# fani-lab/OpeNTF

Measured on AMD Instinct MI355X. Metric: teams/sec (train) bnn_emb d=128 on DBLP, higher is better.
Workload: dtype f32 (fp16x3 split products, f32 accumulate)

## Files before the change

opentf_amd/csrc/ntf_fused_dw.hip:

```cpp
#include "ntf_fused_common.h"

namespace ntf {

struct DwArgs {
    int B, M, Bpad;
    const float *__restrict__ dzT, *__restrict__ h, *__restrict__ hs, *__restrict__ mu, *__restrict__ rho;
    const float* wp;
    const uint32_t* sbits; int nCB; uint32_t so_k0, so_k1; int so_inj;
    float *__restrict__ g_mu, *__restrict__ g_rho, *__restrict__ g_b, *__restrict__ g_bp;
    float klw;
    float *__restrict__ w_mu, *__restrict__ w_rho, *__restrict__ m_mu, *__restrict__ v_mu, *__restrict__ m_rho, *__restrict__ v_rho;
    float lr_over_bc1, b1, b2, eps, bc2_sqrt;
    int wg_begin;
    int* rflag; int rmode;
    const uint32_t* sT;
    const uint32_t* sinT;
    const uint16_t* hb;
    float a_scale, unscale;
    int ksplit; float* part; int64_t slab; int part_row0;
    unsigned long long* stamps;
    int Hr;
    int ntile, stagger;
    NormalSpec cur_eps; int lean;
    int produce; NormalSpec nx_eps; float* nx_wp; uint16_t *nx_pl_wp, *nx_pl_mu; float nx_pscale; double nx_klw; double* nx_kl; int* nx_rflag;
};

__device__ __forceinline__ float adam_update(float p, float g, float& m, float& v, float lr_over_bc1, float b1, float b2, float eps, float bc2_sqrt) {
    adam_step(p, g, m, v, lr_over_bc1, b1, b2, eps, __builtin_amdgcn_rcpf(bc2_sqrt));
    return p;
}

__device__ __forceinline__ uint32_t transpose32(uint32_t a, int il) {
    uint32_t m = 0x0000FFFFu;
#pragma unroll
    for (int j = 16; j != 0; j >>= 1) {
        const uint32_t pv = (uint32_t)__shfl_xor((int)a, j, 64);
        const bool lower = (il & j) == 0;
        const uint32_t lo = lower ? a : pv, hi = lower ? pv : a;
        const uint32_t t = ((lo >> j) ^ hi) & m;
        a ^= lower ? (t << j) : t;
        m ^= m << (j >> 1);
    }
    return a;
}

__device__ __forceinline__ void dw_produce_next(const DwArgs& p, int64_t idx0, const float (&mu4)[4], const float (&rho4)[4], float& kl, float& amax) {
    float z[4], ov[4];
#if defined(DWQ_ABL) && (DWQ_ABL & 2)
    z[0] = z[1] = z[2] = z[3] = 1.f;
#else
    normal4(p.nx_eps, idx0 >> 2, idx0, INT64_MAX, z);
#endif
#pragma unroll
    for (int j = 0; j < 4; ++j) {
        float ls;
        const float sigma = softplus_rho_fast(rho4[j], ls);
        ov[j] = sigma * z[j];
        kl += -ls + 0.5f * (sigma * sigma + mu4[j] * mu4[j]) - 0.5f;
    }
    if (!p.lean) *reinterpret_cast<float4*>(p.nx_wp + idx0) = make_float4(ov[0], ov[1], ov[2], ov[3]);
    const int64_t row = idx0 >> 7; const int j = (int)(idx0 & 127);
    amax = fmaxf(amax, fmaxf(fmaxf(fabsf(ov[0]), fabsf(ov[1])), fmaxf(fabsf(ov[2]), fabsf(ov[3]))));
    amax = fmaxf(amax, fmaxf(fmaxf(fabsf(mu4[0]), fabsf(mu4[1])), fmaxf(fabsf(mu4[2]), fabsf(mu4[3]))));
    planes_store_quad(p.nx_pl_wp, row, j, 128, ov[0], ov[1], ov[2], ov[3], p.nx_pscale);
    planes_store_quad(p.nx_pl_mu, row, j, 128, mu4[0], mu4[1], mu4[2], mu4[3], p.nx_pscale);
}
__device__ __forceinline__ void dw_produce_next_fnn(const DwArgs& p, int64_t idx0, const float (&mu4)[4], float& amax) {
    const int64_t row = idx0 >> 7; const int j = (int)(idx0 & 127);
    amax = fmaxf(amax, fmaxf(fmaxf(fabsf(mu4[0]), fabsf(mu4[1])), fmaxf(fabsf(mu4[2]), fabsf(mu4[3]))));
    planes_store_quad(p.nx_pl_mu, row, j, 128, mu4[0], mu4[1], mu4[2], mu4[3], p.nx_pscale);
}
template <bool BAYES = true>
__device__ __forceinline__ void dw_produce_finish(const DwArgs& p, float kl, float amax, double* red, int nwaves) {
    if (!(amax * p.nx_pscale <= 65504.f)) *p.nx_rflag = 1;
    if (!BAYES) return;
    const double s = wave_reduce_sum_d((double)kl);
    __syncthreads();
    if ((threadIdx.x & 63) == 0) red[threadIdx.x >> 6] = s;
    __syncthreads();
    if (threadIdx.x == 0) { double t = 0.0; for (int w = 0; w < nwaves; ++w) t += red[w]; atomicAdd(p.nx_kl, t * p.nx_klw); }
}

template <int H, bool BAYES, bool ADAM, int HG = H, bool PAD = false>
__device__ __forceinline__ void out_dw_f32_body(const DwArgs& p, char* smem, int jh = 0) {
    constexpr int NJT = H / 32;
    constexpr int KB = 32;
    constexpr int HROW = 4 * H;
    constexpr int TA = DW_TC * KB * 4;
    constexpr int TH = KB * HROW;
    constexpr int STAGE = TA + (BAYES ? 2 : 1) * TH;
    const int tid = threadIdx.x, lane = tid & 63, wave = tid >> 6, il = lane & 31, half = lane >> 5;
    if (range_guard_skip(p.rflag, p.rmode, false)) return;
    const int c0 = (p.wg_begin + blockIdx.x) * DW_TC;
    const int crow = wave * 32 + il;
    const int c = c0 + crow;
    const int nib = p.Bpad / KB;

    f32x16 acc1[NJT], acc2[NJT];
#pragma unroll
    for (int j = 0; j < NJT; ++j)
#pragma unroll
        for (int r = 0; r < 16; ++r) { acc1[j][r] = 0.f; acc2[j][r] = 0.f; }
    float sum1 = 0.f, sum2 = 0.f;

    const uint32_t smem_base = lds_addr(smem);
    const int wave_u = __builtin_amdgcn_readfirstlane(wave);
    auto stage = [&](int ib, int buf) {
        const uint32_t sb = smem_base + buf * STAGE;
#pragma unroll
        for (int n = 0; n < TA / 1024 / DW_WAVES; ++n) {
            const int inst = wave_u * (TA / 1024 / DW_WAVES) + n;
            const int row = inst * 8 + (lane >> 3), pch = lane & 7;
            const int q = pch ^ ((row >> 1) & 7);
            glds16(p.dzT + ((int64_t)(c0 >> 8) * nib + ib) * 8192 + row * 32 + 4 * q, sb + inst * 1024);
        }
        constexpr int HI = TH / 1024;
#pragma unroll
        for (int n = 0; n < (HI + DW_WAVES - 1) / DW_WAVES; ++n) {
            const int inst = wave_u * ((HI + DW_WAVES - 1) / DW_WAVES) + n;
            if (inst < HI) {
                int64_t goff = (int64_t)ib * KB * H + inst * 256 + lane * 4;
                if constexpr (HG != H) { const int f = inst * 256 + lane * 4; goff = (int64_t)(ib * KB + f / H) * HG + jh * H + f % H; }
                glds16(p.h + goff, sb + TA + inst * 1024);
                if (BAYES) glds16(p.hs + goff, sb + TA + TH + inst * 1024);
            }
        }
    };

    const uint32_t cb = (uint32_t)((c0 + wave * 32) >> 5);
    auto sign_col_word = [&](int ib) -> uint32_t {
        const int i = ib * KB + il;
        uint32_t w = 0u;
        if (p.so_inj) { if ((int)cb < p.nCB) w = p.sbits[(int64_t)i * p.nCB + cb]; }
        else w = sign_word(p.so_k0, p.so_k1, (uint32_t)i, cb);
        return transpose32(w, il);
    };
    uint32_t word_next = 0;
    if (BAYES) word_next = sign_col_word(0);
    stage(0, 0);
    asm volatile("s_waitcnt vmcnt(0)" ::: "memory");
    __syncthreads();
    for (int ib = 0; ib < nib; ++ib) {
        const int buf = ib & 1;
        const uint32_t word = word_next >> (4 * half);
        if (BAYES && ib + 1 < nib) word_next = sign_col_word(ib + 1);
        if (ib + 1 < nib) stage(ib + 1, buf ^ 1);
        const char* sA = smem + buf * STAGE;
        const char* sH = sA + TA;
#pragma unroll
        for (int t = 0; t < 4; ++t) {
            const int q = 2 * t + half;
            const float4 a = *reinterpret_cast<const float4*>(sA + crow * 128 + 16 * (q ^ ((crow >> 1) & 7)));
            const float av[4] = {a.x, a.y, a.z, a.w};
#pragma unroll
            for (int e4 = 0; e4 < 4; ++e4) {
                const int kk = 8 * t + e4;
                const float a1 = av[e4];
                sum1 += a1;
                float a2 = a1;
                if (BAYES) { a2 = __uint_as_float(__float_as_uint(a1) ^ ((word << (31 - kk)) & 0x80000000u)); sum2 += a2; }
                const char* hb = sH + (kk + 4 * half) * HROW + 4 * NJT * il;
                float bv[NJT], bsv[NJT];
                if (NJT == 4) {
                    const float4 b4 = *reinterpret_cast<const float4*>(hb); bv[0] = b4.x; bv[1] = b4.y; bv[NJT > 2 ? 2 : 0] = b4.z; bv[NJT > 3 ? 3 : 0] = b4.w;
                    if (BAYES) { const float4 s4 = *reinterpret_cast<const float4*>(hb + TH); bsv[0] = s4.x; bsv[1] = s4.y; bsv[NJT > 2 ? 2 : 0] = s4.z; bsv[NJT > 3 ? 3 : 0] = s4.w; }
                } else if (NJT == 2) {
                    const float2 b2 = *reinterpret_cast<const float2*>(hb); bv[0] = b2.x; bv[NJT > 1 ? 1 : 0] = b2.y;
                    if (BAYES) { const float2 s2 = *reinterpret_cast<const float2*>(hb + TH); bsv[0] = s2.x; bsv[NJT > 1 ? 1 : 0] = s2.y; }
                } else {
                    bv[0] = *reinterpret_cast<const float*>(hb);
                    if (BAYES) bsv[0] = *reinterpret_cast<const float*>(hb + TH);
                }
#pragma unroll
                for (int jt = 0; jt < NJT; ++jt) {
                    acc1[jt] = __builtin_amdgcn_mfma_f32_32x32x2f32(a1, bv[jt], acc1[jt], 0, 0, 0);
                    if (BAYES) acc2[jt] = __builtin_amdgcn_mfma_f32_32x32x2f32(a2, bsv[jt], acc2[jt], 0, 0, 0);
                }
            }
        }
        asm volatile("s_waitcnt vmcnt(0)" ::: "memory");
        __syncthreads();
    }

    sum1 += __shfl_xor(sum1, 32, 64);
    sum2 += __shfl_xor(sum2, 32, 64);
    if (half == 0 && c < p.M && jh == 0) { p.g_b[c] = sum1; if (BAYES) p.g_bp[c] = sum2; }

    float nx_kl = 0.f, nx_amax = 0.f;
    const int ldw = PAD ? p.Hr : HG;
    const bool lane_live = !PAD || jh * H + NJT * il < p.Hr;
#pragma unroll
    for (int r = 0; r < 16; ++r) {
        const int cr = c0 + wave * 32 + rowmap(r, half);
        if (cr >= p.M || !lane_live) continue;
        const int64_t idx0 = (int64_t)cr * ldw + jh * H + NJT * il;
        float gm[NJT], gr[NJT], pm[NJT], pr[NJT];
#pragma unroll
        for (int jt = 0; jt < NJT; ++jt) {
            pm[jt] = ADAM ? p.w_mu[idx0 + jt] : (BAYES ? p.mu[idx0 + jt] : 0.f);
            if (!BAYES) { gm[jt] = acc1[jt][r]; gr[jt] = 0.f; pr[jt] = 0.f; }
            else {
                const float rh = ADAM ? p.w_rho[idx0 + jt] : p.rho[idx0 + jt], w = p.wp[idx0 + jt];
                pr[jt] = rh;
                const RhoTerms t = rho_terms(rh);
                gm[jt] = acc1[jt][r] + p.klw * pm[jt];
                gr[jt] = (t.lo ? acc2[jt][r] * w : acc2[jt][r] * (w / t.sigma) * t.sg) + p.klw * t.kl_a * t.kl_b;
            }
        }
        if (!ADAM) {
#pragma unroll
            for (int jt = 0; jt < NJT; ++jt) { p.g_mu[idx0 + jt] = gm[jt]; if (BAYES) p.g_rho[idx0 + jt] = gr[jt]; }
        } else {
            float nmu[4] = {0.f, 0.f, 0.f, 0.f}, nrho[4] = {0.f, 0.f, 0.f, 0.f};
#pragma unroll
            for (int jt = 0; jt < NJT; ++jt) {
                float m = p.m_mu[idx0 + jt], v = p.v_mu[idx0 + jt];
                nmu[jt & 3] = p.w_mu[idx0 + jt] = adam_update(pm[jt], gm[jt], m, v, p.lr_over_bc1, p.b1, p.b2, p.eps, p.bc2_sqrt);
                p.m_mu[idx0 + jt] = m; p.v_mu[idx0 + jt] = v;
                if (BAYES) {
                    float m2 = p.m_rho[idx0 + jt], v2 = p.v_rho[idx0 + jt];
                    nrho[jt & 3] = p.w_rho[idx0 + jt] = adam_update(pr[jt], gr[jt], m2, v2, p.lr_over_bc1, p.b1, p.b2, p.eps, p.bc2_sqrt);
                    p.m_rho[idx0 + jt] = m2; p.v_rho[idx0 + jt] = v2;
                }
            }
            if constexpr (H == 128 && HG == 128 && !PAD) { if (p.produce) { if constexpr (BAYES) dw_produce_next(p, idx0, nmu, nrho, nx_kl, nx_amax); else dw_produce_next_fnn(p, idx0, nmu, nx_amax); } }
        }
    }
    if constexpr (ADAM && H == 128 && HG == 128 && !PAD) { if (p.produce) dw_produce_finish<BAYES>(p, nx_kl, nx_amax, reinterpret_cast<double*>(smem), DW_WAVES); }
}
// ... 163 lines not shown
        float a_m1[NJT], a_v1[NJT], a_m2[NJT], a_v2[NJT];
        if (ADAM) { ld_vec<NJT>(p.m_mu + idx0, a_m1); ld_vec<NJT>(p.v_mu + idx0, a_v1); if (BAYES) { ld_vec<NJT>(p.m_rho + idx0, a_m2); ld_vec<NJT>(p.v_rho + idx0, a_v2); } }
#pragma unroll
        for (int jt = 0; jt < NJT; ++jt) {
            float gm = acc1[jt][r] * p.unscale, gr = 0.f, pm = 0.f, rh = 0.f;
            if (BAYES) {
                rh = v_rho[jt];
                pm = v_mu[jt];
                const float w = v_wp[jt];
                const RhoTerms t = rho_terms_fast<true>(rh);
                gm += p.klw * pm;
                const float s2 = acc2[jt][r] * p.unscale;
                gr = (t.lo ? s2 * w : s2 * (w * t.isig) * t.sg) + p.klw * t.kl_a * t.kl_b;
            } else if (ADAM) pm = v_mu[jt];
            o_mu[jt] = gm; o_rho[jt] = gr;
            if (ADAM) {
                o_mu[jt] = adam_update(pm, gm, a_m1[jt], a_v1[jt], p.lr_over_bc1, p.b1, p.b2, p.eps, p.bc2_sqrt);
                if (BAYES) o_rho[jt] = adam_update(rh, gr, a_m2[jt], a_v2[jt], p.lr_over_bc1, p.b1, p.b2, p.eps, p.bc2_sqrt);
            }
        }
        if (!ADAM) { st_vec<NJT>(p.g_mu + idx0, o_mu); if (BAYES) st_vec<NJT>(p.g_rho + idx0, o_rho); }
        else {
            st_vec<NJT>(p.w_mu + idx0, o_mu); st_vec<NJT>(p.m_mu + idx0, a_m1); st_vec<NJT>(p.v_mu + idx0, a_v1);
            if (BAYES) { st_vec<NJT>(p.w_rho + idx0, o_rho); st_vec<NJT>(p.m_rho + idx0, a_m2); st_vec<NJT>(p.v_rho + idx0, a_v2); }
        }
    }
}


constexpr int SWT_IB = 16;
__global__ __launch_bounds__(256) void k_sign_words_T(const uint32_t* __restrict__ sbits, int so_inj, uint32_t k0, uint32_t k1, int B, int nCB, int ncb_all, int nib,
                                                      uint32_t* __restrict__ sT) {
    const int lane = threadIdx.x & 63, il = lane & 31, half = lane >> 5;
    const int cb = (blockIdx.x * 4 + (threadIdx.x >> 6)) * 2 + half;
    if (cb >= ncb_all) return;
    const int c = cb * 32 + il;
    uint32_t* dst = sT + (int64_t)(c >> 8) * nib * 256 + (c & 255);
    const int ib_end = min(nib, (int)(blockIdx.y + 1) * SWT_IB);
    for (int ib = blockIdx.y * SWT_IB; ib < ib_end; ++ib) {
        const int i = ib * 32 + il;
        uint32_t w = 0u;
        if (i < B) {
            if (so_inj) { if (cb < nCB) w = sbits[(int64_t)i * nCB + cb]; }
            else w = sign_word(k0, k1, (uint32_t)i, (uint32_t)cb);
        }
        dst[(int64_t)ib * 256] = transpose32(w, il);
    }
}

template <int N> struct DwOps { float rho[N], mu[N], m1[N], v1[N], m2[N], v2[N]; };
template <bool BAYES, bool ADAM, int N>
__device__ __forceinline__ void dw_ops_load(const DwArgs& p, int64_t idx0, DwOps<N>& o) {
    if (BAYES) { ld_vec<N>((ADAM ? p.w_rho : p.rho) + idx0, o.rho); ld_vec<N>((ADAM ? p.w_mu : p.mu) + idx0, o.mu); }
    else if (ADAM) ld_vec<N>(p.w_mu + idx0, o.mu);
    if (ADAM) { ld_vec<N>(p.m_mu + idx0, o.m1); ld_vec<N>(p.v_mu + idx0, o.v1); if (BAYES) { ld_vec<N>(p.m_rho + idx0, o.m2); ld_vec<N>(p.v_rho + idx0, o.v2); } }
}
template <bool BAYES, bool ADAM, int N>
__device__ __forceinline__ void dw_finish_ops(const DwArgs& p, int64_t idx0, const float (&s1)[N], const float (&s2)[N], DwOps<N>& o, float& nx_kl, float& nx_amax) {
    static_assert(N == 4, "one Philox quad per call");
    float o_mu[N], o_rho[N], z[4] = {0.f, 0.f, 0.f, 0.f};
#if defined(DWQ_ABL) && (DWQ_ABL & 1)
    z[0] = z[1] = z[2] = z[3] = 1.f;
#else
    if (BAYES) normal4(p.cur_eps, idx0 >> 2, idx0, INT64_MAX, z);
#endif
#pragma unroll
    for (int jt = 0; jt < N; ++jt) {
        float gm = s1[jt], gr = 0.f, pm = 0.f, rh = 0.f;
        if (BAYES) {
            rh = o.rho[jt];
            pm = o.mu[jt];
            const RhoTerms t = rho_terms_fast<true>(rh);
            gm += p.klw * pm;
            gr = s2[jt] * z[jt] * t.sg + p.klw * t.kl_a * t.kl_b;
        } else if (ADAM) pm = o.mu[jt];
        o_mu[jt] = gm; o_rho[jt] = gr;
        if (ADAM) {
            o_mu[jt] = adam_update(pm, gm, o.m1[jt], o.v1[jt], p.lr_over_bc1, p.b1, p.b2, p.eps, p.bc2_sqrt);
            if (BAYES) o_rho[jt] = adam_update(rh, gr, o.m2[jt], o.v2[jt], p.lr_over_bc1, p.b1, p.b2, p.eps, p.bc2_sqrt);
        }
    }
    if (!ADAM) { st_vec<N>(p.g_mu + idx0, o_mu); if (BAYES) st_vec<N>(p.g_rho + idx0, o_rho); }
    else {
        st_vec<N>(p.w_mu + idx0, o_mu); st_vec<N>(p.m_mu + idx0, o.m1); st_vec<N>(p.v_mu + idx0, o.v1);
        if (BAYES) { st_vec<N>(p.w_rho + idx0, o_rho); st_vec<N>(p.m_rho + idx0, o.m2); st_vec<N>(p.v_rho + idx0, o.v2); }
        if constexpr (N == 4) { if (p.produce) { if constexpr (BAYES) dw_produce_next(p, idx0, o_mu, o_rho, nx_kl, nx_amax); else dw_produce_next_fnn(p, idx0, o_mu, nx_amax); } }
    }
}
template <bool BAYES, bool ADAM, int N>
__device__ __forceinline__ void dw_finish_vec(const DwArgs& p, int64_t idx0, const float (&s1)[N], const float (&s2)[N], float& nx_kl, float& nx_amax) {
    DwOps<N> o;
    dw_ops_load<BAYES, ADAM, N>(p, idx0, o);
    dw_finish_ops<BAYES, ADAM, N>(p, idx0, s1, s2, o, nx_kl, nx_amax);
}

template <bool BAYES, bool ADAM>
__global__ __launch_bounds__(256) void k_out_dw_finish(DwArgs p) {
    if (p.rflag && *p.rflag) return;
    const int64_t q = (int64_t)blockIdx.x * 256 + threadIdx.x, il0 = q * 4, idx0 = il0 + (int64_t)p.part_row0 * 128;
    const int64_t Mp = p.slab / 128;
    if (q < Mp && q + p.part_row0 < p.M) {
        const float* pb = p.part + (int64_t)p.ksplit * 2 * p.slab;
        float b1 = 0.f, b2 = 0.f;
        for (int s = 0; s < p.ksplit; ++s) { b1 += pb[(int64_t)(s * 2) * Mp + q]; if (BAYES) b2 += pb[(int64_t)(s * 2 + 1) * Mp + q]; }
        p.g_b[q + p.part_row0] = b1; if (BAYES) p.g_bp[q + p.part_row0] = b2;
    }
    float nx_kl = 0.f, nx_amax = 0.f;
    const bool produce = ADAM && p.produce;
    const bool live = il0 < p.slab && idx0 < (int64_t)p.M * 128;
    if (!live && !produce) return;
    float s1[4] = {0.f, 0.f, 0.f, 0.f}, s2[4] = {0.f, 0.f, 0.f, 0.f};
    if (live) {
    for (int s = 0; s < p.ksplit; ++s) {
        float t[4];
        ld_vec<4>(p.part + (int64_t)(s * 2) * p.slab + il0, t);
#pragma unroll
        for (int k = 0; k < 4; ++k) s1[k] += t[k];
        if (BAYES) {
            ld_vec<4>(p.part + (int64_t)(s * 2 + 1) * p.slab + il0, t);
#pragma unroll
            for (int k = 0; k < 4; ++k) s2[k] += t[k];
        }
    }
    dw_finish_vec<BAYES, ADAM, 4>(p, idx0, s1, s2, nx_kl, nx_amax);
    }
    if (produce) { __shared__ double red[4]; dw_produce_finish<BAYES>(p, nx_kl, nx_amax, red, 4); }
}

__host__ __device__ __forceinline__ int sin_word_bit(int r) { const int g = r >> 3, q = (r & 7) >> 1, o = r & 1; return 16 * o + 4 * g + 3 - q; }
__global__ void k_sin_words_T(const uint32_t* __restrict__ sinbits, int Bpad, uint32_t* __restrict__ sinT) {
    const int t = blockIdx.x * blockDim.x + threadIdx.x;
    if (t >= (Bpad >> 5) * 128) return;
    const int ib = t >> 7, j = t & 127;
    uint32_t w = 0u;
    for (int r = 0; r < 32; ++r) w |= ((sinbits[(int64_t)(ib * 32 + r) * 4 + (j >> 5)] >> (j & 31)) & 1u) << sin_word_bit(r);
    sinT[t] = w;
}

#ifndef DW_EPI_PD
#define DW_EPI_PD 1
#endif
#ifndef DWQ_PRIO
#define DWQ_PRIO 2
#endif
#ifndef DWQ_BRING
#define DWQ_BRING 2
#endif
#ifndef DWQ_PPG
#define DWQ_PPG 3
#endif
constexpr int QW = 4;
constexpr int QTC = 32 * QW;
template <bool BAYES, bool ADAM, bool STAMP = false, bool SPLIT = false>
__global__ __launch_bounds__(64 * QW, 2) void k_out_dw_q(DwArgs p) {
    extern __shared__ __attribute__((aligned(16))) char smem[];
    constexpr int H = 128, NJT = 4;
    constexpr int TA = QTC * 32 * 4;
    constexpr int PLANE = H * 64;
    constexpr int TB = 2 * PLANE;
    constexpr int SRC_TB = (BAYES ? 2 : 1) * TB;
    constexpr int TW = BAYES ? 1024 : 0;
    constexpr int STAGE = TA + TB + TW;
    typedef _Float16 h2_t __attribute__((ext_vector_type(2)));
    const int tid = threadIdx.x, lane = tid & 63, wave = tid >> 6, il = lane & 31, half = lane >> 5;
    if (p.rmode == 1 && __builtin_nontemporal_load(p.rflag) != 0) return;
    const int ntile_s = SPLIT ? (int)gridDim.x / p.ksplit : 0;
    const int ksi = SPLIT ? (int)blockIdx.x / ntile_s : 0;
    const int c0 = (p.wg_begin + (SPLIT ? (int)blockIdx.x % ntile_s : (int)blockIdx.x)) * QTC;
    const int crow = wave * 32 + il, c = c0 + crow;
    const int nib = p.Bpad / 32;
    const int ib0 = SPLIT ? (int)((int64_t)ksi * nib / p.ksplit) : 0, ib1 = SPLIT ? (int)((int64_t)(ksi + 1) * nib / p.ksplit) : nib;
    const uint32_t smem_base = lds_addr(smem);
    const int wave_u = __builtin_amdgcn_readfirstlane(wave);
    const char* hb = reinterpret_cast<const char*>(p.hb);
    unsigned long long st_t[4] = {0, 0, 0, 0};
    if (STAMP) st_t[0] = __builtin_amdgcn_s_memrealtime();
    uint32_t lds_base = 0u;
    if (STAMP || (p.stagger > 0 && (int)blockIdx.x < p.ntile)) asm volatile("s_getreg_b32 %0, hwreg(HW_REG_LDS_ALLOC, 0, 8)" : "=s"(lds_base));
    if (p.stagger > 0 && (int)blockIdx.x < p.ntile) {
        if (lds_base != 0u) {
            const uint64_t t0 = __builtin_amdgcn_s_memrealtime();
            while (__builtin_amdgcn_s_memrealtime() - t0 < (uint64_t)p.stagger) __builtin_amdgcn_s_sleep(64);
        }
    }

    const h2_t ones = {(_Float16)1.0f, (_Float16)1.0f};
    constexpr int NA = TA / 1024 / QW, NB = TB / 1024 / QW;
    const float* dz_tile = p.dzT + (int64_t)(c0 >> 8) * nib * 8192 + ((c0 & 255) << 5);
    const uint32_t* sw_src = BAYES ? (half == 0 ? p.sT + (int64_t)(c0 >> 8) * nib * 256 + (c0 & 255) + il * 4 : p.sinT + il * 4) : nullptr;
    const int sw_step = half == 0 ? 256 : 128;
    auto stage_piece = [&](int ib, int buf, int n) {
        const uint32_t sb = smem_base + buf * STAGE;
        if (n < NA) {
            const int inst = wave_u * NA + n;
            const int row = inst * 8 + (lane >> 3), pch = lane & 7;
            const int q = pch ^ ((row >> 1) & 7);
            glds16(dz_tile + (int64_t)ib * 8192 + row * 32 + 4 * q, sb + inst * 1024);
        } else {
            const char* src = hb + (size_t)ib * SRC_TB;
            const int inst = wave_u * NB + (n - NA);
            const int pos = inst * 1024 + lane * 16;
            const int j = (pos % PLANE) >> 6, cd = (pos >> 4) & 3;
            glds16(src + (pos & ~63) + 16 * (cd ^ ((j >> 2) & 3)), sb + TA + inst * 1024);
            if (BAYES && n == NA + NB - 1) glds16(sw_src + (int64_t)ib * sw_step, sb + TA + TB);
        }
    };
    float nx_kl = 0.f, nx_amax = 0.f;
    unsigned long long st_c[3] = {0, 0, 0}, c_prev = 0;
    auto cyc = [&]() -> unsigned long long {
        unsigned long long t;
        __builtin_amdgcn_sched_barrier(0);
        asm volatile("s_memtime %0\n\ts_waitcnt lgkmcnt(0)" : "=s"(t) :: "memory");
        __builtin_amdgcn_sched_barrier(0);
        return t;
    };
#pragma unroll
    for (int n = 0; n < NA + NB; ++n) stage_piece(ib0, 0, n);
    f32x16 acc1[NJT], acc2[NJT];
#pragma unroll
    for (int j = 0; j < NJT; ++j)
#pragma unroll
        for (int r = 0; r < 16; ++r) { acc1[j][r] = 0.f; acc2[j][r] = 0.f; }
    float sum1 = 0.f, sum2 = 0.f;
    const int shl0 = 12 - 4 * half, shl1 = 4 - 4 * half;
    asm volatile("s_waitcnt vmcnt(0)" ::: "memory");
    __syncthreads();
    auto k_block = [&](int ib, auto more_c) {
        constexpr bool MORE = decltype(more_c)::value;
        const int buf = (ib - ib0) & 1;
        const char* sA = smem + buf * STAGE;
        const char* sB = sA + TA;
        uint32_t word = 0u;
        u32x4 iw = {0u, 0u, 0u, 0u};
        if (BAYES) { word = *reinterpret_cast<const uint32_t*>(sA + TA + TB + crow * 4); iw = *reinterpret_cast<const u32x4*>(sA + TA + TB + 512 + il * 16); }
        constexpr int NG = 2 * NJT;
        const char* bbase = sB + il * 64;
        const int swz = (il >> 2) & 3;
        auto load_b = [&](int g, u32x4 (&dst)[2]) {
            const int ks = g / NJT, jt = g % NJT;
            const char* bp = bbase + jt * 2048 + 16 * ((2 * ks + half) ^ swz);
#pragma unroll
            for (int q = 0; q < 2; ++q) dst[q] = *reinterpret_cast<const u32x4*>(bp + q * PLANE);
        };
        u32x4 a[2][2], as[2][2];
        auto prep_a = [&](int ks) {
            const int ch = 4 * ks + 2 * half, sw = (crow >> 1) & 7;
            const u32x4 lo = *reinterpret_cast<const u32x4*>(sA + crow * 128 + 16 * (ch ^ sw));
            const u32x4 hi = *reinterpret_cast<const u32x4*>(sA + crow * 128 + 16 * ((ch + 1) ^ sw));
            const uint32_t x[8] = {lo[0], lo[1], lo[2], lo[3], hi[0], hi[1], hi[2], hi[3]};
            const uint32_t w8 = word >> (ks * 16 + half * 8);
#pragma unroll
            for (int q = 0; q < 4; ++q) {
                const uint32_t p1 = __builtin_amdgcn_perm(x[2 * q + 1], x[2 * q], 0x05040100u), p2 = __builtin_amdgcn_perm(x[2 * q + 1], x[2 * q], 0x07060302u);
                a[ks][0][q] = p1; a[ks][1][q] = p2;
                sum1 = __builtin_amdgcn_fdot2(__builtin_bit_cast(h2_t, p1), ones, sum1, false);
                sum1 = __builtin_amdgcn_fdot2(__builtin_bit_cast(h2_t, p2), ones, sum1, false);
                if (BAYES) {
                    const uint32_t m = ((w8 << (15 - 2 * q)) & 0x8000u) | ((w8 << (30 - 2 * q)) & 0x80000000u);
                    const uint32_t s1 = p1 ^ m, s2 = p2 ^ m;
                    as[ks][0][q] = s1; as[ks][1][q] = s2;
                    sum2 = __builtin_amdgcn_fdot2(__builtin_bit_cast(h2_t, s1), ones, sum2, false);
                    sum2 = __builtin_amdgcn_fdot2(__builtin_bit_cast(h2_t, s2), ones, sum2, false);
                }
            }
        };
        constexpr int BR = DWQ_BRING;
        u32x4 bq[BR][2], bs[2];
#pragma unroll
        for (int g = 0; g < BR - 1; ++g) load_b(g, bq[g]);
        prep_a(0);
        int piece = 0;
        auto dma = [&]() {
            if (MORE) {
#pragma unroll
                for (int q = 0; q < DWQ_PPG; ++q) { if (piece < NA + NB) stage_piece(ib + 1, buf ^ 1, piece); ++piece; }
            }
        };
#pragma unroll
        for (int g = 0; g < NG; ++g) {
            if (g + BR - 1 < NG) load_b(g + BR - 1, bq[(g + BR - 1) % BR]);
            asm volatile("" ::: "memory");
            const int ks = g / NJT, jt = g % NJT;
            acc1[jt] = mfma3h(a[ks], bq[g % BR], acc1[jt]);
            dma();
            if (BAYES) {
                const uint32_t v = iw[jt] << (ks ? shl1 : shl0);
#pragma unroll
                for (int q = 0; q < 4; ++q) {
                    const uint32_t m = (v << q) & 0x80008000u;
                    bs[0][q] = bq[g % BR][0][q] ^ m; bs[1][q] = bq[g % BR][1][q] ^ m;
                }
                acc2[jt] = mfma3h(as[ks], bs, acc2[jt]);
                dma();
            }
            if (g == 0) prep_a(1);
        }
        if (STAMP) { st_c[0] += cyc() - c_prev; c_prev = cyc(); }
        asm volatile("s_waitcnt vmcnt(0)" ::: "memory");
        if (STAMP) { st_c[1] += cyc() - c_prev; c_prev = cyc(); }
        __syncthreads();
        if (STAMP) { st_c[2] += cyc() - c_prev; c_prev = cyc(); }
    };
    if (STAMP) { st_t[1] = __builtin_amdgcn_s_memrealtime(); c_prev = cyc(); }
    if (DWQ_PRIO) __builtin_amdgcn_s_setprio(DWQ_PRIO);
    for (int ib = ib0; ib < ib1 - 1; ++ib) k_block(ib, std::true_type{});
    k_block(ib1 - 1, std::false_type{});
    if (DWQ_PRIO) __builtin_amdgcn_s_setprio(0);
    if (STAMP) st_t[2] = __builtin_amdgcn_s_memrealtime();
    sum1 += __shfl_xor(sum1, 32, 64);
    sum2 += __shfl_xor(sum2, 32, 64);
    const float inv_a = 1.f / p.a_scale;
    if constexpr (SPLIT) {
        if (half == 0 && c < p.M) {
            float* pb = p.part + (int64_t)p.ksplit * 2 * p.slab; const int64_t Mp = p.slab / 128; const int cl = c - p.part_row0;
            pb[(int64_t)(ksi * 2) * Mp + cl] = sum1 * inv_a; if (BAYES) pb[(int64_t)(ksi * 2 + 1) * Mp + cl] = sum2 * inv_a;
        }
#pragma unroll
        for (int r = 0; r < 16; ++r) {
            const int cr = c0 + wave * 32 + rowmap(r, half);
            if (cr >= p.M) continue;
            const int64_t il0 = (int64_t)(cr - p.part_row0) * H + NJT * il;
            float s1[NJT], s2[NJT];
#pragma unroll
            for (int jt = 0; jt < NJT; ++jt) { s1[jt] = acc1[jt][r] * p.unscale; s2[jt] = acc2[jt][r] * p.unscale; }
            st_vec<NJT>(p.part + (int64_t)(ksi * 2) * p.slab + il0, s1);
            if (BAYES) st_vec<NJT>(p.part + (int64_t)(ksi * 2 + 1) * p.slab + il0, s2);
        }
        return;
    }
    if (half == 0 && c < p.M) { p.g_b[c] = sum1 * inv_a; if (BAYES) p.g_bp[c] = sum2 * inv_a; }

    constexpr int PD = DW_EPI_PD;
    DwOps<NJT> ops[PD + 1];
    auto row_idx = [&](int r, int64_t& idx0) -> bool {
        const int cr = c0 + wave * 32 + rowmap(r, half);
        idx0 = (int64_t)cr * H + NJT * il;
        return cr < p.M;
    };
    static_for<0, PD>([&](auto rc) { constexpr int r = decltype(rc)::value; int64_t idx0; if (row_idx(r, idx0)) dw_ops_load<BAYES, ADAM, NJT>(p, idx0, ops[r % (PD + 1)]); });
    static_for<0, 16>([&](auto rc) {
        constexpr int r = decltype(rc)::value;
        if constexpr (r + PD < 16) { int64_t idn; if (row_idx(r + PD, idn)) dw_ops_load<BAYES, ADAM, NJT>(p, idn, ops[(r + PD) % (PD + 1)]); }
        int64_t idx0;
        if (row_idx(r, idx0)) {
            float s1[NJT], s2[NJT];
#pragma unroll
            for (int jt = 0; jt < NJT; ++jt) { s1[jt] = acc1[jt][r] * p.unscale; s2[jt] = acc2[jt][r] * p.unscale; }
            dw_finish_ops<BAYES, ADAM, NJT>(p, idx0, s1, s2, ops[r % (PD + 1)], nx_kl, nx_amax);
        }
    });
    if (STAMP && p.stamps && lane == 0) {
        asm volatile("s_waitcnt vmcnt(0)" ::: "memory");
        st_t[3] = __builtin_amdgcn_s_memrealtime();
        uint32_t hw_id, xcc;
        asm volatile("s_getreg_b32 %0, hwreg(HW_REG_HW_ID)" : "=s"(hw_id));
        asm volatile("s_getreg_b32 %0, hwreg(HW_REG_XCC_ID)" : "=s"(xcc));
        unsigned long long* o = p.stamps + ((int64_t)blockIdx.x * QW + wave) * 10;
        o[0] = st_t[0]; o[1] = st_t[1]; o[2] = st_t[2]; o[3] = st_t[3]; o[4] = ((unsigned long long)xcc << 32) | hw_id; o[5] = lds_base;
        o[6] = st_c[0]; o[7] = st_c[1]; o[8] = st_c[2]; o[9] = 0;
    }
    if (ADAM && p.produce) dw_produce_finish<BAYES>(p, nx_kl, nx_amax, reinterpret_cast<double*>(smem + 2 * STAGE), QW);
}

void launch_fused_out_dw(hipStream_t st, const FusedDw& f) {
    const Geom g = geom(f.B, f.M);
    const WsLayout w = ws_layout(f.B, f.H, f.M);
    char* ws = static_cast<char*>(f.ws);
    DwArgs a;
    a.B = f.B; a.M = f.M; a.Bpad = g.Bpad; a.dzT = f.dzT; a.h = reinterpret_cast<const float*>(ws + w.hz); a.hs = reinterpret_cast<const float*>(ws + w.hs);
    a.mu = f.mu; a.rho = f.rho; a.wp = f.wp; a.sbits = reinterpret_cast<const uint32_t*>(ws + w.sbits); a.nCB = g.nCB;
    a.so_k0 = f.s_out.k0; a.so_k1 = f.s_out.k1; a.so_inj = f.s_out_inj;
    a.g_mu = f.g_mu; a.g_rho = f.g_rho; a.g_b = f.g_b; a.g_bp = f.g_bp; a.klw = f.klw;
    a.w_mu = f.w_mu; a.w_rho = f.w_rho; a.m_mu = f.m_mu; a.v_mu = f.v_mu; a.m_rho = f.m_rho; a.v_rho = f.v_rho;
    a.lr_over_bc1 = f.lr_over_bc1; a.b1 = f.b1; a.b2 = f.b2; a.eps = f.eps; a.bc2_sqrt = f.bc2_sqrt;
    const int total = (f.M + DW_TC - 1) / DW_TC;
    const int grid = f.wg_count > 0 ? std::min(f.wg_count, total - f.wg_begin) : total;
    a.wg_begin = f.wg_count > 0 ? f.wg_begin : 0;
    if (grid <= 0) return;
    a.hb = reinterpret_cast<const uint16_t*>(ws + w.hb);
    a.rflag = f.rflag; a.rmode = 0;
    a.produce = (f.produce && f.adam && f.H == 128) ? 1 : 0;
    a.cur_eps = f.cur_eps; a.lean = (a.produce && f.lean) ? 1 : 0;
    a.nx_eps = f.nx_eps; a.nx_wp = f.nx_wp; a.nx_pl_wp = f.nx_pl_wp; a.nx_pl_mu = f.nx_pl_mu; a.nx_pscale = f.nx_pscale; a.nx_klw = f.nx_klw; a.nx_kl = f.nx_kl; a.nx_rflag = f.nx_rflag;
    a.ntile = 0; a.stagger = 0; a.stamps = nullptr;
    const bool guard = f.split && f.rflag != nullptr;
    a.sT = reinterpret_cast<const uint32_t*>(ws + w.sbitsT);
    a.ksplit = 1; a.part = nullptr; a.slab = 0; a.part_row0 = 0;
    const int Ht = fused_tmpl(f.H);
    const bool pad = Ht != f.H;
    a.Hr = f.H;
    if (Ht == 256) {
        const size_t lds = 2 * ((size_t)DW_TC * 32 * 4 + (size_t)(f.bayes ? 2 : 1) * 32 * 4 * 128);
#define NTF_DWH(BY, AD) do { auto kf = k_out_dw_h2<BY, AD>; set_max_lds(reinterpret_cast<const void*>(kf), (int)lds);              \
        hipLaunchKernelGGL(kf, dim3(grid, 2), dim3(64 * DW_WAVES), lds, st, a); } while (0)
#define NTF_DWHP(BY, AD) do { auto kf = k_out_dw_h2<BY, AD, true>; set_max_lds(reinterpret_cast<const void*>(kf), (int)lds);       \
        hipLaunchKernelGGL(kf, dim3(grid, 2), dim3(64 * DW_WAVES), lds, st, a); } while (0)
        if (pad) { if (f.bayes) { if (f.adam) NTF_DWHP(true, true); else NTF_DWHP(true, false); } else { if (f.adam) NTF_DWHP(false, true); else NTF_DWHP(false, false); } }
        else
        if (f.bayes) { if (f.adam) NTF_DWH(true, true); else NTF_DWH(true, false); } else { if (f.adam) NTF_DWH(false, true); else NTF_DWH(false, false); }
#undef NTF_DWHP
#undef NTF_DWH
        return;
    }
    if (pad) {
        const size_t lds = 2 * ((size_t)DW_TC * 32 * 4 + (size_t)(f.bayes ? 2 : 1) * 32 * 4 * 128);
#define NTF_DWP(BY, AD) do { auto kf = k_out_dw<128, BY, AD, true>; set_max_lds(reinterpret_cast<const void*>(kf), (int)lds);      \
        hipLaunchKernelGGL(kf, dim3(grid), dim3(64 * DW_WAVES), lds, st, a); } while (0)
        if (f.bayes) { if (f.adam) NTF_DWP(true, true); else NTF_DWP(true, false); } else { if (f.adam) NTF_DWP(false, true); else NTF_DWP(false, false); }
#undef NTF_DWP
        return;
    }
    if (f.split && f.dz_packed) {
        a.a_scale = f.a_scale; a.unscale = 1.f / (f.a_scale * f.h_scale); a.rmode = guard ? 1 : 0;
        const int ks = (f.ksplit > 1 && f.part) ? std::min(f.ksplit, std::max(1, g.Bpad / 32)) : 1;
        if (ks > 1) {
            a.sinT = reinterpret_cast<const uint32_t*>(ws + w.sinT);
            const int total_q = (f.M + QTC - 1) / QTC, qb = f.wg_count > 0 ? 2 * f.wg_begin : 0;
            const int qgrid = f.wg_count > 0 ? std::min(2 * f.wg_count, total_q - qb) : total_q;
            const int wg256 = a.wg_begin;
            a.wg_begin = qb;
            a.ksplit = ks; a.part = f.part; a.slab = (int64_t)qgrid * QTC * 128; a.part_row0 = qb * QTC;
            const size_t ldsq = 2 * ((size_t)QTC * 128 + 2 * 128 * 64 + (f.bayes ? 1024 : 0)) + 64;
            const int64_t nq = (int64_t)qgrid * QTC * 128 / 4;
#define NTF_DWQS(BY, AD) do { auto kf = k_out_dw_q<BY, false, false, true>;                                                    \
            set_max_lds(reinterpret_cast<const void*>(kf), (int)ldsq);     \
            hipLaunchKernelGGL(kf, dim3(qgrid * ks), dim3(64 * QW), ldsq, st, a);                                              \
            hipLaunchKernelGGL((k_out_dw_finish<BY, AD>), dim3((unsigned)((nq + 255) / 256)), dim3(256), 0, st, a); } while (0)
            if (f.bayes) { if (f.adam) NTF_DWQS(true, true); else NTF_DWQS(true, false); } else { if (f.adam) NTF_DWQS(false, true); else NTF_DWQS(false, false); }
#undef NTF_DWQS
            if (!guard) return;
            a.rmode = 2; a.ksplit = 1; a.wg_begin = wg256; a.part_row0 = 0;
            goto exact_f32;
        }
        {
            a.sinT = reinterpret_cast<const uint32_t*>(ws + w.sinT);
            const int total_q = (f.M + QTC - 1) / QTC, qb = f.wg_count > 0 ? 2 * f.wg_begin : 0;
            const int qgrid = f.wg_count > 0 ? std::min(2 * f.wg_count, total_q - qb) : total_q;
            const int wg256 = a.wg_begin;
            a.wg_begin = qb;
            static int n_cu = 0;
            if (!n_cu) { int dev = 0; hipGetDevice(&dev); hipDeviceGetAttribute(&n_cu, hipDeviceAttributeMultiprocessorCount, dev); if (n_cu <= 0) n_cu = 256; }
            static const int stagger_q = getenv("NTF_DW_STAGGER") ? atoi(getenv("NTF_DW_STAGGER")) : -1;
            const int nib = g.Bpad / 32;
            a.ntile = 2 * n_cu;
            a.stagger = (f.adam && qgrid > n_cu) ? (stagger_q >= 0 ? stagger_q : (nib * 140 + 4500) / 2) : 0;
            const size_t ldsq = 2 * ((size_t)QTC * 128 + 2 * 128 * 64 + (f.bayes ? 1024 : 0)) + 64;
#define NTF_DWQ(BY, AD) do { auto kf = k_out_dw_q<BY, AD>;                                                                     \
            set_max_lds(reinterpret_cast<const void*>(kf), (int)ldsq);     \
            hipLaunchKernelGGL(kf, dim3(qgrid), dim3(64 * QW), ldsq, st, a); } while (0)
#ifdef NTF_DIAG
            static const char* stamp_file = getenv("NTF_DW_STAMP_FILE");
#else
            static const char* stamp_file = nullptr;
#endif
            if (stamp_file && f.bayes && f.adam) {
                static unsigned long long* d_st = nullptr; static int n_launch = 0;
                if (!d_st) hipMalloc(&d_st, (size_t)qgrid * QW * 10 * 8);
                a.stamps = d_st;
                auto kf = k_out_dw_q<true, true, true>;
                set_max_lds(reinterpret_cast<const void*>(kf), (int)ldsq);
                hipLaunchKernelGGL(kf, dim3(qgrid), dim3(64 * QW), ldsq, st, a);
                if (++n_launch == 30) {
                    std::vector<unsigned long long> hst((size_t)qgrid * QW * 10);
                    hipStreamSynchronize(st); hipMemcpy(hst.data(), d_st, hst.size() * 8, hipMemcpyDeviceToHost);
                    if (FILE* fp = fopen(stamp_file, "wb")) { fwrite(hst.data(), 8, hst.size(), fp); fclose(fp); }
                }
            }
            else if (f.bayes) { if (f.adam) NTF_DWQ(true, true); else NTF_DWQ(true, false); } else { if (f.adam) NTF_DWQ(false, true); else NTF_DWQ(false, false); }
#undef NTF_DWQ
            if (!guard) return;
            a.rmode = 2; a.wg_begin = wg256; a.ntile = 0; a.stagger = 0;
            goto exact_f32;
        }
    }
    if (f.split) {
        a.rmode = guard ? 1 : 0;
        a.a_scale = f.a_scale; a.unscale = 1.f / (f.a_scale * f.h_scale);
#define NTF_DWB1(HH, BY, AD) do { auto kf = k_out_dw_b6<HH, BY, AD>; const size_t lds = 2 * ((size_t)DW_TC * 128 + (size_t)(BY ? 2 : 1) * 2 * HH * 64); \
        set_max_lds(reinterpret_cast<const void*>(kf), (int)lds);                                      \
        hipLaunchKernelGGL(kf, dim3(grid), dim3(64 * DW_WAVES), lds, st, a); } while (0)
#define NTF_DWB(HH) do { if (f.bayes) { if (f.adam) NTF_DWB1(HH, true, true); else NTF_DWB1(HH, true, false); }                                            \
                         else { if (f.adam) NTF_DWB1(HH, false, true); else NTF_DWB1(HH, false, false); } } while (0)
        if (f.H == 128) NTF_DWB(128); else if (f.H == 64) NTF_DWB(64); else NTF_DWB(32);
#undef NTF_DWB
#undef NTF_DWB1
        if (!guard) return;
        a.rmode = 2;
    }
exact_f32:
    a.ntile = grid;
#define NTF_DW1(HH, BY) do { const bool fb = a.rmode == 2;                                                                                    \
        auto kf = fb ? (f.adam ? k_out_dw_fallback<HH, BY, true> : k_out_dw_fallback<HH, BY, false>) : (f.adam ? k_out_dw<HH, BY, true> : k_out_dw<HH, BY, false>);   \
        const size_t lds = 2 * (DW_TC * 32 * 4 + (BY ? 2 : 1) * 32 * 4 * HH);                                                                \
        set_max_lds(reinterpret_cast<const void*>(kf), (int)lds);                      \
        hipLaunchKernelGGL(kf, dim3(fb ? std::min(grid, 256) : grid), dim3(64 * DW_WAVES), lds, st, a); } while (0)
#define NTF_DW(HH) do { if (f.bayes) NTF_DW1(HH, true); else NTF_DW1(HH, false); } while (0)
    if (f.H == 128) NTF_DW(128); else if (f.H == 64) NTF_DW(64); else NTF_DW(32);
#undef NTF_DW
}

void launch_fused_prep_planes(hipStream_t st, int B, int H, int M, int bayes, void* ws_, float h_scale, const SignSpec* s_out, int s_out_inj, int which) {
    const Geom g = geom(B, M);
    const WsLayout w = ws_layout(B, H, M);
    char* ws = static_cast<char*>(ws_);
    if (bayes && s_out && (which & 1)) {
        const int ncb_all = rup(M, DW_TC) / 32, nib = g.Bpad / 32;
        hipLaunchKernelGGL(k_sign_words_T, dim3((ncb_all + 7) / 8, (nib + SWT_IB - 1) / SWT_IB), dim3(256), 0, st, reinterpret_cast<const uint32_t*>(ws + w.sbits), s_out_inj, s_out->k0, s_out->k1,
                           B, g.nCB, ncb_all, nib, reinterpret_cast<uint32_t*>(ws + w.sbitsT));
    }
    if (!(which & 2)) return;
    const int n = g.Bpad * H;
    hipLaunchKernelGGL(k_prep_planes_T, dim3((n + 255) / 256), dim3(256), 0, st, reinterpret_cast<const float*>(ws + w.hz), reinterpret_cast<const float*>(ws + w.hs),
                       bayes, g.Bpad, H, h_scale, reinterpret_cast<uint16_t*>(ws + w.hb));
    if (bayes && H == 128)
        hipLaunchKernelGGL(k_sin_words_T, dim3((g.Bpad / 32 * 128 + 255) / 256), dim3(256), 0, st, reinterpret_cast<const uint32_t*>(ws + w.sinbits), g.Bpad, reinterpret_cast<uint32_t*>(ws + w.sinT));
}

}
```

profiles/dw_stamps.py:

```python
import numpy as np, sys
a = np.fromfile(sys.argv[1], dtype=np.uint64).reshape(-1, 4, 10)
w0 = a[:, 0, :]
t0 = w0[:, 0].min()
ent = (w0[:, 0] - t0) / 100.0; mb = (w0[:, 1] - t0) / 100.0; me = (w0[:, 2] - t0) / 100.0; ex = (w0[:, 3] - t0) / 100.0
hw = w0[:, 4] & 0xffffffff; xcc = w0[:, 4] >> 32; lds = w0[:, 5]
cu = ((xcc.astype(np.int64) & 15) << 8) | ((hw.astype(np.int64) >> 8) & 0xff)
print("workgroups", len(w0), "distinct CUs", len(np.unique(cu)), "kernel span us", ex.max())
print("lds_base values", np.unique(lds, return_counts=True))
print("first-round (first 512) lds_base != 0:", int((lds[:512] != 0).sum()))
print("main loop us: mean %.1f  p10 %.1f p90 %.1f | epilogue us: mean %.1f p10 %.1f p90 %.1f | stagger wait mean %.1f" % (
    (me - mb).mean(), np.percentile(me - mb, 10), np.percentile(me - mb, 90), (ex - me).mean(), np.percentile(ex - me, 10), np.percentile(ex - me, 90), (mb - ent).mean()))
tot_ov = 0.0; tot_main2 = 0.0; tot_epi2 = 0.0; tot = 0.0
for c in np.unique(cu):
    idx = np.where(cu == c)[0]
    ev = []
    for i in idx: ev += [(mb[i], 'm', 1), (me[i], 'm', -1), (me[i], 'e', 1), (ex[i], 'e', -1)]
    ev.sort()
    nm = ne = 0; last = ev[0][0]
    for t, k, d in ev:
        dt = t - last; last = t
        if nm >= 1 and ne >= 1: tot_ov += dt
        if nm >= 2: tot_main2 += dt
        if ne >= 2: tot_epi2 += dt
        tot += dt
        if k == 'm': nm += d
        else: ne += d
print("cycles per K block and wave (all waves): body %.0f | DMA wait %.0f | barrier %.0f" % tuple(a[:, :, 6 + k].mean() / 32 for k in range(3)))
print("per-CU time: main||epilogue %.1f %%  two main loops %.1f %%  two epilogues %.1f %%" % (100 * tot_ov / tot, 100 * tot_main2 / tot, 100 * tot_epi2 / tot))
c = np.unique(cu)[3]
idx = np.where(cu == c)[0]; idx = idx[np.argsort(ent[idx])]
print("CU", hex(c))
for i in idx: print("  wg %5d lds %3d enter %7.1f main %7.1f..%7.1f exit %7.1f" % (i, lds[i], ent[i], mb[i], me[i], ex[i]))
```

Baseline: 697,800.

## Make quantized dW kernel persistent and prefetch next tile during epilogue

Converts k_out_dw_q into a persistent kernel: the grid is capped at two workgroups per CU (or NTF_DW_SLOTS), and each workgroup loops over column tiles with a stride of the grid size. The first K-block of the next tile is staged into LDS before the current tile's epilogue, so that load overlaps the Adam/produce epilogue. Kernel args are reloaded from the kernarg segment to ease register pressure, the LDS swizzle address math is simplified with glds16s offsets, and KL is accumulated in double across tiles. This trades per-workgroup launch and ramp cost for a longer-lived workgroup with more live state.

After: 686,400. -1.6%, worse.

```diff
diff --git a/opentf_amd/csrc/ntf_fused_dw.hip b/opentf_amd/csrc/ntf_fused_dw.hip
--- a/opentf_amd/csrc/ntf_fused_dw.hip
+++ b/opentf_amd/csrc/ntf_fused_dw.hip
@@ -71,10 +71,10 @@
     planes_store_quad(p.nx_pl_mu, row, j, 128, mu4[0], mu4[1], mu4[2], mu4[3], p.nx_pscale);
 }
 template <bool BAYES = true>
-__device__ __forceinline__ void dw_produce_finish(const DwArgs& p, float kl, float amax, double* red, int nwaves) {
+__device__ __forceinline__ void dw_produce_finish(const DwArgs& p, double kl, float amax, double* red, int nwaves) {
     if (!(amax * p.nx_pscale <= 65504.f)) *p.nx_rflag = 1;
     if (!BAYES) return;
-    const double s = wave_reduce_sum_d((double)kl);
+    const double s = wave_reduce_sum_d(kl);
     __syncthreads();
     if ((threadIdx.x & 63) == 0) red[threadIdx.x >> 6] = s;
     __syncthreads();
@@ -544,7 +544,10 @@
 constexpr int QW = 4;
 constexpr int QTC = 32 * QW;
 template <bool BAYES, bool ADAM, bool STAMP = false, bool SPLIT = false>
-__global__ __launch_bounds__(64 * QW, 2) void k_out_dw_q(DwArgs p) {
+__global__ __launch_bounds__(64 * QW, 2) void k_out_dw_q(DwArgs p_) {
+    typedef const __attribute__((address_space(4))) DwArgs* kargs_t;
+    kargs_t pk = (kargs_t)__builtin_amdgcn_kernarg_segment_ptr();
+    DwArgs p = *(const DwArgs*)pk;
     extern __shared__ __attribute__((aligned(16))) char smem[];
     constexpr int H = 128, NJT = 4;
     constexpr int TA = QTC * 32 * 4;
@@ -554,22 +557,23 @@
     constexpr int TW = BAYES ? 1024 : 0;
     constexpr int STAGE = TA + TB + TW;
     typedef _Float16 h2_t __attribute__((ext_vector_type(2)));
-    const int tid = threadIdx.x, lane = tid & 63, wave = tid >> 6, il = lane & 31, half = lane >> 5;
+    int tid = threadIdx.x, lane = tid & 63, wave = tid >> 6, il = lane & 31, half = lane >> 5;
     if (p.rmode == 1 && __builtin_nontemporal_load(p.rflag) != 0) return;
     const int ntile_s = SPLIT ? (int)gridDim.x / p.ksplit : 0;
     const int ksi = SPLIT ? (int)blockIdx.x / ntile_s : 0;
-    const int c0 = (p.wg_begin + (SPLIT ? (int)blockIdx.x % ntile_s : (int)blockIdx.x)) * QTC;
-    const int crow = wave * 32 + il, c = c0 + crow;
+    const int t_first = SPLIT ? (int)blockIdx.x % ntile_s : (int)blockIdx.x;
+    const int t_end = SPLIT ? t_first + 1 : p.ntile, t_step = SPLIT ? 1 : (int)gridDim.x;
+    int crow = wave * 32 + il;
     const int nib = p.Bpad / 32;
     const int ib0 = SPLIT ? (int)((int64_t)ksi * nib / p.ksplit) : 0, ib1 = SPLIT ? (int)((int64_t)(ksi + 1) * nib / p.ksplit) : nib;
     const uint32_t smem_base = lds_addr(smem);
-    const int wave_u = __builtin_amdgcn_readfirstlane(wave);
+    int wave_u = __builtin_amdgcn_readfirstlane(wave);
     const char* hb = reinterpret_cast<const char*>(p.hb);
     unsigned long long st_t[4] = {0, 0, 0, 0};
     if (STAMP) st_t[0] = __builtin_amdgcn_s_memrealtime();
     uint32_t lds_base = 0u;
-    if (STAMP || (p.stagger > 0 && (int)blockIdx.x < p.ntile)) asm volatile("s_getreg_b32 %0, hwreg(HW_REG_LDS_ALLOC, 0, 8)" : "=s"(lds_base));
-    if (p.stagger > 0 && (int)blockIdx.x < p.ntile) {
+    if (STAMP || p.stagger > 0) asm volatile("s_getreg_b32 %0, hwreg(HW_REG_LDS_ALLOC, 0, 8)" : "=s"(lds_base));
+    if (p.stagger > 0) {
         if (lds_base != 0u) {
             const uint64_t t0 = __builtin_amdgcn_s_memrealtime();
             while (__builtin_amdgcn_s_memrealtime() - t0 < (uint64_t)p.stagger) __builtin_amdgcn_s_sleep(64);
@@ -578,26 +582,25 @@
 
     const h2_t ones = {(_Float16)1.0f, (_Float16)1.0f};
     constexpr int NA = TA / 1024 / QW, NB = TB / 1024 / QW;
-    const float* dz_tile = p.dzT + (int64_t)(c0 >> 8) * nib * 8192 + ((c0 & 255) << 5);
-    const uint32_t* sw_src = BAYES ? (half == 0 ? p.sT + (int64_t)(c0 >> 8) * nib * 256 + (c0 & 255) + il * 4 : p.sinT + il * 4) : nullptr;
-    const int sw_step = half == 0 ? 256 : 128;
-    auto stage_piece = [&](int ib, int buf, int n) {
+    static_assert(NA % 2 == 0 && PLANE == 8192, "stage_piece's lane offsets");
+    auto stage_piece = [&](int tc0, int ib, int buf, int n) {
+        const float* dz_tile = p.dzT + (int64_t)(tc0 >> 8) * nib * 8192 + ((tc0 & 255) << 5);
+        const uint32_t* sw_src = BAYES ? (half == 0 ? p.sT + (int64_t)(tc0 >> 8) * nib * 256 + (tc0 & 255) + il * 4 : p.sinT + il * 4) : nullptr;
         const uint32_t sb = smem_base + buf * STAGE;
         if (n < NA) {
             const int inst = wave_u * NA + n;
-            const int row = inst * 8 + (lane >> 3), pch = lane & 7;
-            const int q = pch ^ ((row >> 1) & 7);
-            glds16(dz_tile + (int64_t)ib * 8192 + row * 32 + 4 * q, sb + inst * 1024);
+            const int rl = lane >> 3, pch = lane & 7;
+            const int q = pch ^ (4 * (n & 1) + (rl >> 1));
+            glds16s(dz_tile + (int64_t)ib * 8192 + inst * 256, (uint32_t)(rl * 32 + 4 * q) * 4u, sb + inst * 1024);
         } else {
             const char* src = hb + (size_t)ib * SRC_TB;
             const int inst = wave_u * NB + (n - NA);
-            const int pos = inst * 1024 + lane * 16;
-            const int j = (pos % PLANE) >> 6, cd = (pos >> 4) & 3;
-            glds16(src + (pos & ~63) + 16 * (cd ^ ((j >> 2) & 3)), sb + TA + inst * 1024);
-            if (BAYES && n == NA + NB - 1) glds16(sw_src + (int64_t)ib * sw_step, sb + TA + TB);
+            glds16s(src + inst * 1024, (uint32_t)((lane >> 2) * 64 + 16 * ((lane & 3) ^ ((lane >> 4) & 3))), sb + TA + inst * 1024);
+            if (BAYES && n == NA + NB - 1) glds16(sw_src + (int64_t)ib * (half == 0 ? 256 : 128), sb + TA + TB);
         }
     };
-    float nx_kl = 0.f, nx_amax = 0.f;
+    double nx_kl_d = 0.0;
+    float nx_amax = 0.f;
     unsigned long long st_c[3] = {0, 0, 0}, c_prev = 0;
     auto cyc = [&]() -> unsigned long long {
         unsigned long long t;
@@ -606,15 +609,23 @@
         __builtin_amdgcn_sched_barrier(0);
         return t;
     };
-#pragma unroll
-    for (int n = 0; n < NA + NB; ++n) stage_piece(ib0, 0, n);
+    const float inv_a = 1.f / p.a_scale;
+#pragma unroll
+    for (int n = 0; n < NA + NB; ++n) stage_piece((p.wg_begin + t_first) * QTC, ib0, 0, n);
+    for (int t = t_first; t < t_end; t += t_step) {
+    asm volatile("" : "+v"(tid));
+    lane = tid & 63; wave = tid >> 6; il = lane & 31; half = lane >> 5; crow = wave * 32 + il; wave_u = __builtin_amdgcn_readfirstlane(wave);
+    const int shl0 = 12 - 4 * half, shl1 = 4 - 4 * half;
+    int c0 = (p.wg_begin + t) * QTC;
+    int c = c0 + crow;
+    if (STAMP && t != t_first) { st_t[0] = __builtin_amdgcn_s_memrealtime(); st_c[0] = st_c[1] = st_c[2] = 0; }
+    float nx_kl = 0.f;
     f32x16 acc1[NJT], acc2[NJT];
 #pragma unroll
     for (int j = 0; j < NJT; ++j)
 #pragma unroll
         for (int r = 0; r < 16; ++r) { acc1[j][r] = 0.f; acc2[j][r] = 0.f; }
     float sum1 = 0.f, sum2 = 0.f;
-    const int shl0 = 12 - 4 * half, shl1 = 4 - 4 * half;
     asm volatile("s_waitcnt vmcnt(0)" ::: "memory");
     __syncthreads();
     auto k_block = [&](int ib, auto more_c) {
@@ -665,7 +676,7 @@
         auto dma = [&]() {
             if (MORE) {
 #pragma unroll
-                for (int q = 0; q < DWQ_PPG; ++q) { if (piece < NA + NB) stage_piece(ib + 1, buf ^ 1, piece); ++piece; }
+                for (int q = 0; q < DWQ_PPG; ++q) { if (piece < NA + NB) stage_piece(c0, ib + 1, buf ^ 1, piece); ++piece; }
             }
         };
 #pragma unroll
@@ -699,9 +710,15 @@
     k_block(ib1 - 1, std::false_type{});
     if (DWQ_PRIO) __builtin_amdgcn_s_setprio(0);
     if (STAMP) st_t[2] = __builtin_amdgcn_s_memrealtime();
+    if constexpr (!SPLIT) {
+        if (t + t_step < t_end) {
+            int cn = (p.wg_begin + t + t_step) * QTC;
+#pragma unroll
+            for (int n = 0; n < NA + NB; ++n) stage_piece(cn, 0, 0, n);
+        }
+    }
     sum1 += __shfl_xor(sum1, 32, 64);
     sum2 += __shfl_xor(sum2, 32, 64);
-    const float inv_a = 1.f / p.a_scale;
     if constexpr (SPLIT) {
         if (half == 0 && c < p.M) {
             float* pb = p.part + (int64_t)p.ksplit * 2 * p.slab; const int64_t Mp = p.slab / 128; const int cl = c - p.part_row0;
@@ -720,10 +737,15 @@
         }
         return;
     }
+    asm volatile("" : "+s"(pk));
+    p = *(const DwArgs*)pk;
+    asm volatile("" : "+v"(tid));
+    lane = tid & 63; wave = tid >> 6; il = lane & 31; half = lane >> 5; crow = wave * 32 + il;
+    c = c0 + crow;
     if (half == 0 && c < p.M) { p.g_b[c] = sum1 * inv_a; if (BAYES) p.g_bp[c] = sum2 * inv_a; }
 
     constexpr int PD = DW_EPI_PD;
-    DwOps<NJT> ops[PD + 1];
+    DwOps<NJT> ops[PD + 1] = {};
     auto row_idx = [&](int r, int64_t& idx0) -> bool {
         const int cr = c0 + wave * 32 + rowmap(r, half);
         idx0 = (int64_t)cr * H + NJT * il;
@@ -747,11 +769,13 @@
         uint32_t hw_id, xcc;
         asm volatile("s_getreg_b32 %0, hwreg(HW_REG_HW_ID)" : "=s"(hw_id));
         asm volatile("s_getreg_b32 %0, hwreg(HW_REG_XCC_ID)" : "=s"(xcc));
-        unsigned long long* o = p.stamps + ((int64_t)blockIdx.x * QW + wave) * 10;
+        unsigned long long* o = p.stamps + ((int64_t)t * QW + wave) * 10;
         o[0] = st_t[0]; o[1] = st_t[1]; o[2] = st_t[2]; o[3] = st_t[3]; o[4] = ((unsigned long long)xcc << 32) | hw_id; o[5] = lds_base;
-        o[6] = st_c[0]; o[7] = st_c[1]; o[8] = st_c[2]; o[9] = 0;
-    }
-    if (ADAM && p.produce) dw_produce_finish<BAYES>(p, nx_kl, nx_amax, reinterpret_cast<double*>(smem + 2 * STAGE), QW);
+        o[6] = st_c[0]; o[7] = st_c[1]; o[8] = st_c[2]; o[9] = blockIdx.x;
+    }
+    nx_kl_d += (double)nx_kl;
+    }
+    if (ADAM && p.produce) dw_produce_finish<BAYES>(p, nx_kl_d, nx_amax, reinterpret_cast<double*>(smem + 2 * STAGE), QW);
 }
 
 void launch_fused_out_dw(hipStream_t st, const FusedDw& f) {
@@ -833,13 +857,15 @@
             static int n_cu = 0;
             if (!n_cu) { int dev = 0; hipGetDevice(&dev); hipDeviceGetAttribute(&n_cu, hipDeviceAttributeMultiprocessorCount, dev); if (n_cu <= 0) n_cu = 256; }
             static const int stagger_q = getenv("NTF_DW_STAGGER") ? atoi(getenv("NTF_DW_STAGGER")) : -1;
+            static const int slots_q = getenv("NTF_DW_SLOTS") ? atoi(getenv("NTF_DW_SLOTS")) : 0;
             const int nib = g.Bpad / 32;
-            a.ntile = 2 * n_cu;
-            a.stagger = (f.adam && qgrid > n_cu) ? (stagger_q >= 0 ? stagger_q : (nib * 140 + 4500) / 2) : 0;
+            const int wgrid = std::min(qgrid, slots_q > 0 ? slots_q : 2 * n_cu);
+            a.ntile = qgrid;
+            a.stagger = (f.adam && wgrid > n_cu) ? (stagger_q >= 0 ? stagger_q : (nib * 140 + 4500) / 2) : 0;
             const size_t ldsq = 2 * ((size_t)QTC * 128 + 2 * 128 * 64 + (f.bayes ? 1024 : 0)) + 64;
 #define NTF_DWQ(BY, AD) do { auto kf = k_out_dw_q<BY, AD>;                                                                     \
             set_max_lds(reinterpret_cast<const void*>(kf), (int)ldsq);     \
-            hipLaunchKernelGGL(kf, dim3(qgrid), dim3(64 * QW), ldsq, st, a); } while (0)
+            hipLaunchKernelGGL(kf, dim3(wgrid), dim3(64 * QW), ldsq, st, a); } while (0)
 #ifdef NTF_DIAG
             static const char* stamp_file = getenv("NTF_DW_STAMP_FILE");
 #else
@@ -851,7 +877,7 @@
                 a.stamps = d_st;
                 auto kf = k_out_dw_q<true, true, true>;
                 set_max_lds(reinterpret_cast<const void*>(kf), (int)ldsq);
-                hipLaunchKernelGGL(kf, dim3(qgrid), dim3(64 * QW), ldsq, st, a);
+                hipLaunchKernelGGL(kf, dim3(wgrid), dim3(64 * QW), ldsq, st, a);
                 if (++n_launch == 30) {
                     std::vector<unsigned long long> hst((size_t)qgrid * QW * 10);
                     hipStreamSynchronize(st); hipMemcpy(hst.data(), d_st, hst.size() * 8, hipMemcpyDeviceToHost);
diff --git a/profiles/dw_stamps.py b/profiles/dw_stamps.py
--- a/profiles/dw_stamps.py
+++ b/profiles/dw_stamps.py
@@ -5,7 +5,7 @@
 ent = (w0[:, 0] - t0) / 100.0; mb = (w0[:, 1] - t0) / 100.0; me = (w0[:, 2] - t0) / 100.0; ex = (w0[:, 3] - t0) / 100.0
 hw = w0[:, 4] & 0xffffffff; xcc = w0[:, 4] >> 32; lds = w0[:, 5]
 cu = ((xcc.astype(np.int64) & 15) << 8) | ((hw.astype(np.int64) >> 8) & 0xff)
-print("workgroups", len(w0), "distinct CUs", len(np.unique(cu)), "kernel span us", ex.max())
+print("half-tiles", len(w0), "distinct CUs", len(np.unique(cu)), "kernel span us", ex.max())
 print("lds_base values", np.unique(lds, return_counts=True))
 print("first-round (first 512) lds_base != 0:", int((lds[:512] != 0).sum()))
 print("main loop us: mean %.1f  p10 %.1f p90 %.1f | epilogue us: mean %.1f p10 %.1f p90 %.1f | stagger wait mean %.1f" % (
@@ -27,7 +27,18 @@
         else: ne += d
 print("cycles per K block and wave (all waves): body %.0f | DMA wait %.0f | barrier %.0f" % tuple(a[:, :, 6 + k].mean() / 32 for k in range(3)))
 print("per-CU time: main||epilogue %.1f %%  two main loops %.1f %%  two epilogues %.1f %%" % (100 * tot_ov / tot, 100 * tot_main2 / tot, 100 * tot_epi2 / tot))
+gaps = []; per_slot = []
+for key in set(zip(cu.tolist(), lds.tolist())):
+    idx = np.where((cu == key[0]) & (lds == key[1]))[0]; idx = idx[np.argsort(mb[idx])]
+    g = mb[idx[1:]] - ex[idx[:-1]]
+    gaps += g.tolist(); per_slot.append((len(idx), ex[idx].max() - mb[idx].min(), g.sum()))
+gaps = np.array(gaps); per_slot = np.array(per_slot)
+if len(gaps):
+    print("between tiles on a slot (exit -> next main-loop begin) us: mean %.1f  p10 %.1f  p50 %.1f  p90 %.1f  max %.1f  (%d gaps on %d slots)" % (
+        gaps.mean(), np.percentile(gaps, 10), np.percentile(gaps, 50), np.percentile(gaps, 90), gaps.max(), len(gaps), len(per_slot)))
+    print("per slot: tiles mean %.2f | first main-loop begin -> last exit us mean %.1f | of which between tiles mean %.1f" % (per_slot[:, 0].mean(), per_slot[:, 1].mean(), per_slot[:, 2].mean()))
+print("per tile us (main-loop begin -> exit): mean %.1f" % (ex - mb).mean())
 c = np.unique(cu)[3]
 idx = np.where(cu == c)[0]; idx = idx[np.argsort(ent[idx])]
 print("CU", hex(c))
-for i in idx: print("  wg %5d lds %3d enter %7.1f main %7.1f..%7.1f exit %7.1f" % (i, lds[i], ent[i], mb[i], me[i], ex[i]))
+for i in idx: print("  tile %5d wg %5d lds %3d enter %7.1f main %7.1f..%7.1f exit %7.1f" % (i, w0[i, 9], lds[i], ent[i], mb[i], me[i], ex[i]))
```
